# pierreaubert/math-audio

Hardware: NVIDIA B200
Metric: bem_assemble_plus_gmres_seconds_per_frequency (lower is better)
Workload: dtype f64

## Files before the change

### math_audio_b200/csrc/linalg.cu

```cuda
#include <cooperative_groups.h>
#include <atomic>
#include <cstdlib>

#include <string>

#include "linalg.h"

namespace cg = cooperative_groups;

namespace bemb {

constexpr int MAX_DEVICES = 64;
static inline int cur_dev() {
    int d = 0;
    if (cudaGetDevice(&d) != cudaSuccess) { cudaGetLastError(); d = 0; }
    return d >= 0 && d < MAX_DEVICES ? d : MAX_DEVICES - 1;
}
struct PerDeviceFlag {
    std::atomic<unsigned char> v[MAX_DEVICES];
    PerDeviceFlag() { for (auto& x : v) x.store(0); }
    bool get() const { return v[cur_dev()].load() != 0; }
    void set() { v[cur_dev()].store(1); }
};
struct PerDeviceInt {
    std::atomic<int> v[MAX_DEVICES];
    explicit PerDeviceInt(int init) { for (auto& x : v) x.store(init); }
    int get() const { return v[cur_dev()].load(); }
    void set(int val) { v[cur_dev()].store(val); }
};

namespace {

constexpr int GEMV_THREADS = 256;

__device__ __forceinline__ double2 ld_stream(const cplx* p) { return __ldcs(reinterpret_cast<const double2*>(p)); }
__device__ __forceinline__ double2 ld_ro(const cplx* p) { return __ldg(reinterpret_cast<const double2*>(p)); }

__device__ __forceinline__ void cfma(double& are, double& aim, double2 a, double2 x) {
    are = fma(a.x, x.x, are);
    are = fma(-a.y, x.y, are);
    aim = fma(a.x, x.y, aim);
    aim = fma(a.y, x.x, aim);
}

__device__ __forceinline__ unsigned long long global_timer_ns() {
    unsigned long long t;
    asm volatile("mov.u64 %0, %globaltimer;" : "=l"(t));
    return t;
}
__device__ __forceinline__ void ll_store(uint4* dst, double re, double im, uint32_t flag) {
    const uint32_t rl = (uint32_t)__double2loint(re), rh = (uint32_t)__double2hiint(re);
    const uint32_t il = (uint32_t)__double2loint(im), ih = (uint32_t)__double2hiint(im);
    asm volatile("st.volatile.global.v4.u32 [%0], {%1, %2, %3, %4};" ::"l"(dst), "r"(rl), "r"(flag), "r"(rh), "r"(flag) : "memory");
    asm volatile("st.volatile.global.v4.u32 [%0], {%1, %2, %3, %4};" ::"l"(dst + 1), "r"(il), "r"(flag), "r"(ih), "r"(flag) : "memory");
}
template <int N>
__device__ __forceinline__ void ll_load_many(cplx (&out)[N], const uint4* src, uint64_t first, uint64_t stride, uint64_t len,
                                             uint32_t flag, int* err, unsigned long long timeout_ns) {
    bool have[N];
#pragma unroll
    for (int e = 0; e < N; ++e) {
        have[e] = first + (uint64_t)e * stride >= len;
        out[e] = C(0, 0);
    }
    unsigned long long t0 = 0;
    unsigned int spins = 0;
    for (;;) {
        uint4 a[N], b[N];
#pragma unroll
        for (int e = 0; e < N; ++e) {
            if (!have[e]) {
                const uint4* q = src + 2 * (first + (uint64_t)e * stride);
                asm volatile("ld.volatile.global.v4.u32 {%0, %1, %2, %3}, [%4];" : "=r"(a[e].x), "=r"(a[e].y), "=r"(a[e].z), "=r"(a[e].w) : "l"(q) : "memory");
                asm volatile("ld.volatile.global.v4.u32 {%0, %1, %2, %3}, [%4];" : "=r"(b[e].x), "=r"(b[e].y), "=r"(b[e].z), "=r"(b[e].w) : "l"(q + 1) : "memory");
            }
        }
        bool all = true;
#pragma unroll
        for (int e = 0; e < N; ++e) {
            if (!have[e]) {
                if (a[e].y == flag && a[e].w == flag && b[e].y == flag && b[e].w == flag) {
                    have[e] = true;
                    out[e] = C(__hiloint2double((int)a[e].z, (int)a[e].x), __hiloint2double((int)b[e].z, (int)b[e].x));
                } else {
                    all = false;
                }
            }
        }
        if (all) break;
        if ((++spins & 63u) == 0) {
            const unsigned long long t = global_timer_ns();
            if (t0 == 0) t0 = t;
            else if (t - t0 > timeout_ns) {
                *reinterpret_cast<volatile int*>(err) = 1;
                break;
            }
        }
    }
}

template <int GEMV_RB, int GEMV_U, bool FUSED>
__global__ void __launch_bounds__(GEMV_THREADS)
zgemv_kernel(const cplx* __restrict__ A, uint64_t lda, uint64_t nrows, uint64_t ncols, const cplx* __restrict__ x,
             cplx* __restrict__ y, PeerOut po) {
    __shared__ double red[GEMV_RB][2][GEMV_THREADS / 32];
    const int tid = threadIdx.x, lane = tid & 31, warp = tid >> 5;
    for (uint64_t rb = (uint64_t)blockIdx.x * GEMV_RB; rb < nrows; rb += (uint64_t)gridDim.x * GEMV_RB) {
        double are[GEMV_RB], aim[GEMV_RB];
        const cplx* rowp[GEMV_RB];
#pragma unroll
        for (int r = 0; r < GEMV_RB; ++r) {
            are[r] = 0.0; aim[r] = 0.0;
            uint64_t row = rb + r < nrows ? rb + r : nrows - 1;
            rowp[r] = A + row * lda;
        }
        uint64_t c = tid;
        for (; c + (GEMV_U - 1) * GEMV_THREADS < ncols; c += GEMV_U * GEMV_THREADS) {
            double2 a[GEMV_RB][GEMV_U], xv[GEMV_U];
#pragma unroll
            for (int u = 0; u < GEMV_U; ++u) {
#pragma unroll
                for (int r = 0; r < GEMV_RB; ++r) a[r][u] = ld_stream(rowp[r] + c + u * GEMV_THREADS);
                xv[u] = ld_ro(x + c + u * GEMV_THREADS);
            }
#pragma unroll
            for (int u = 0; u < GEMV_U; ++u)
#pragma unroll
                for (int r = 0; r < GEMV_RB; ++r) cfma(are[r], aim[r], a[r][u], xv[u]);
        }
        for (; c < ncols; c += GEMV_THREADS) {
            const double2 x0 = ld_ro(x + c);
#pragma unroll
            for (int r = 0; r < GEMV_RB; ++r) cfma(are[r], aim[r], ld_stream(rowp[r] + c), x0);
        }
#pragma unroll
        for (int r = 0; r < GEMV_RB; ++r) {
#pragma unroll
            for (int m = 16; m >= 1; m >>= 1) {
                are[r] += __shfl_xor_sync(0xffffffffu, are[r], m);
                aim[r] += __shfl_xor_sync(0xffffffffu, aim[r], m);
            }
            if (lane == 0) { red[r][0][warp] = are[r]; red[r][1][warp] = aim[r]; }
        }
        __syncthreads();
        if (tid < GEMV_RB && rb + tid < nrows) {
            double sr = 0.0, si = 0.0;
#pragma unroll
            for (int w = 0; w < GEMV_THREADS / 32; ++w) { sr += red[tid][0][w]; si += red[tid][1][w]; }
            if (FUSED) {
#pragma unroll
                for (int p = 0; p < MAX_PEERS; ++p)
                    if (p < po.npeers) ll_store(po.ll[p] + 2 * (rb + tid), sr, si, po.epoch);
            } else {
                y[rb + tid] = C(sr, si);
            }
        }
        __syncthreads();
    }
}

constexpr int GEMVT_MAX_CHUNKS = 32;
__global__ void __launch_bounds__(256)
zgemv_t_partial_kernel(const cplx* __restrict__ A, uint64_t lda, uint64_t nrows, uint64_t ncols, uint64_t rows_per_chunk,
                       const cplx* __restrict__ x, cplx* __restrict__ part) {
    const uint64_t col = (uint64_t)blockIdx.x * 256 + threadIdx.x;
    const uint64_t r0 = (uint64_t)blockIdx.y * rows_per_chunk;
    const uint64_t r1 = r0 + rows_per_chunk < nrows ? r0 + rows_per_chunk : nrows;
    if (col >= ncols) return;
    double sr = 0.0, si = 0.0;
    for (uint64_t r = r0; r < r1; ++r) cfma(sr, si, ld_stream(A + r * lda + col), ld_ro(x + r));
    part[(uint64_t)blockIdx.y * ncols + col] = C(sr, si);
}
__global__ void __launch_bounds__(256)
zgemv_t_reduce_kernel(const cplx* __restrict__ part, uint64_t ncols, int nchunks, cplx* __restrict__ y) {
    const uint64_t col = (uint64_t)blockIdx.x * 256 + threadIdx.x;
    if (col >= ncols) return;
    double sr = 0.0, si = 0.0;
    for (int c = 0; c < nchunks; ++c) { sr += part[(uint64_t)c * ncols + col].re; si += part[(uint64_t)c * ncols + col].im; }
    y[col] = C(sr, si);
}

constexpr int MAX_CLUSTER = 16;
constexpr int MAX_WARPS = 32;

struct ClusterShared {
    cplx part[2][MAX_CLUSTER * MAX_WARPS];
};

__device__ __forceinline__ cplx cluster_allreduce(cplx v, ClusterShared& sh, int parity) {
    cg::cluster_group cluster = cg::this_cluster();
    const unsigned nb = cluster.num_blocks(), me = cluster.block_rank();
    const unsigned lane = threadIdx.x & 31, warp = threadIdx.x >> 5, nw = blockDim.x >> 5;
#pragma unroll
    for (int m = 16; m >= 1; m >>= 1) {
        v.re += __shfl_xor_sync(0xffffffffu, v.re, m);
        v.im += __shfl_xor_sync(0xffffffffu, v.im, m);
    }
    if (lane < nb) {
        ClusterShared* remote = cluster.map_shared_rank(&sh, lane);
        remote->part[parity][me * nw + warp] = v;
    }
    cluster.sync();
    cplx t = C(0, 0);
    const unsigned total = nb * nw;
    for (unsigned sidx = lane; sidx < total; sidx += 32) {
        t.re += sh.part[parity][sidx].re;
        t.im += sh.part[parity][sidx].im;
    }
#pragma unroll
    for (int m = 16; m >= 1; m >>= 1) {
        t.re += __shfl_xor_sync(0xffffffffu, t.re, m);
        t.im += __shfl_xor_sync(0xffffffffu, t.im, m);
    }
    return t;
}

__device__ __forceinline__ cplx ldg_c(const cplx* p) {
    double2 v = __ldg(reinterpret_cast<const double2*>(p));
    return C(v.x, v.y);
}

template <int EPT>
__global__ void __launch_bounds__(256)
mgs_cluster_reg_kernel(const cplx* __restrict__ V, uint64_t ldv, const cplx* __restrict__ w, int j, uint64_t n, uint64_t S,
                       cplx* __restrict__ hcol, cplx* __restrict__ vnext, double breakdown_tol,
                       const cplx* __restrict__ pinv, int direct_scale) {
    __shared__ ClusterShared sh;
    cg::cluster_group cluster = cg::this_cluster();
    const unsigned me = cluster.block_rank();
    const uint64_t begin = (uint64_t)me * S;
    const uint64_t end = begin + S < n ? begin + S : n;
    const uint64_t len = end > begin ? end - begin : 0;
    cplx wr[EPT], vc[EPT], vn[EPT];
#pragma unroll
    for (int e = 0; e < EPT; ++e) {
        const uint64_t k = threadIdx.x + (uint64_t)e * blockDim.x;
        wr[e] = k < len ? w[begin + k] : C(0, 0);
        if (pinv && k < len) wr[e] = wr[e] * ldg_c(pinv + begin + k);
        vc[e] = k < len ? ldg_c(V + begin + k) : C(0, 0);
    }
    int parity = 0;
    for (int i = 0; i <= j; ++i) {
        if (i < j) {
            const cplx* vi1 = V + (uint64_t)(i + 1) * ldv + begin;
#pragma unroll
            for (int e = 0; e < EPT; ++e) {
                const uint64_t k = threadIdx.x + (uint64_t)e * blockDim.x;
                vn[e] = k < len ? ldg_c(vi1 + k) : C(0, 0);
            }
        }
        cplx acc = C(0, 0);
#pragma unroll
        for (int e = 0; e < EPT; ++e) {
            acc.re = fma(vc[e].re, wr[e].re, fma(vc[e].im, wr[e].im, acc.re));
            acc.im = fma(vc[e].re, wr[e].im, fma(-vc[e].im, wr[e].re, acc.im));
        }
        const cplx h = cluster_allreduce(acc, sh, parity);
        parity ^= 1;
        if (me == 0 && threadIdx.x == 0) hcol[i] = h;
#pragma unroll
        for (int e = 0; e < EPT; ++e) {
            wr[e].re = fma(-h.re, vc[e].re, fma(h.im, vc[e].im, wr[e].re));
            wr[e].im = fma(-h.re, vc[e].im, fma(-h.im, vc[e].re, wr[e].im));
            vc[e] = vn[e];
        }
    }
    cplx acc = C(0, 0);
#pragma unroll
    for (int e = 0; e < EPT; ++e) acc.re = fma(wr[e].re, wr[e].re, fma(wr[e].im, wr[e].im, acc.re));
    const cplx nn = cluster_allreduce(acc, sh, parity);
    const double nrm = sqrt(nn.re);
    if (me == 0 && threadIdx.x == 0) hcol[j + 1] = C(nrm, 0.0);
    if (!(nrm < breakdown_tol)) {
        const double inv = 1.0 / nrm;
        const double sc = inv - 1.0;
#pragma unroll
        for (int e = 0; e < EPT; ++e) {
            const uint64_t k = threadIdx.x + (uint64_t)e * blockDim.x;
            if (k < len)
                vnext[begin + k] = direct_scale ? C(wr[e].re * inv, wr[e].im * inv)
                                                : C(wr[e].re + wr[e].re * sc, wr[e].im + wr[e].im * sc);
        }
    }
    cluster.sync();
}

constexpr int LS_THREADS = 256;
constexpr int LS_WARPS = LS_THREADS / 32;
constexpr int LS_MAXV = 64;

template <int EPT>
__global__ void __launch_bounds__(LS_THREADS)
mgs_lowsync_kernel(const cplx* __restrict__ V, uint64_t ldv, const cplx* __restrict__ w, int j, uint64_t n, uint64_t S,
                   cplx* __restrict__ Lmat, int ldl, cplx* __restrict__ hcol, cplx* __restrict__ vnext, double breakdown_tol,
                   const cplx* __restrict__ pinv, int direct_scale, cplx* __restrict__ hcol_host, PeerWait pw) {
    extern __shared__ __align__(16) unsigned char dyn[];
    __shared__ ClusterShared sh1;
    cplx* warp_part = reinterpret_cast<cplx*>(dyn);
    cplx* slots = warp_part + LS_WARPS * 2 * LS_MAXV;
    cplx* avec = slots + MAX_CLUSTER * 2 * LS_MAXV;
    cplx* Ls = avec + LS_MAXV;
    cg::cluster_group cluster = cg::this_cluster();
    const unsigned nb = cluster.num_blocks(), me = cluster.block_rank();
    const int tid = threadIdx.x, lane = tid & 31, warp = tid >> 5;
    const int nv = j + 1;
    const uint64_t begin = (uint64_t)me * S;
    const uint64_t end = begin + S < n ? begin + S : n;
    const uint64_t len = end > begin ? end - begin : 0;

    cplx wr[EPT], vj[EPT];
    if (pw.ll) ll_load_many<EPT>(wr, pw.ll + 2 * begin, (uint64_t)tid, (uint64_t)LS_THREADS, len, pw.epoch, pw.err, pw.timeout_ns);
#pragma unroll
    for (int e = 0; e < EPT; ++e) {
        const uint64_t k = tid + (uint64_t)e * LS_THREADS;
        if (!pw.ll) wr[e] = k < len ? w[begin + k] : C(0, 0);
        if (pinv && k < len) wr[e] = wr[e] * ldg_c(pinv + begin + k);
        vj[e] = (k < len) ? ldg_c(V + (uint64_t)j * ldv + begin + k) : C(0, 0);
    }
    for (int idx = tid; idx < nv * nv; idx += LS_THREADS) {
        const int k = idx / nv, l = idx - k * nv;
        Ls[idx] = (l < k && k < j) ? Lmat[k * ldl + l] : C(0, 0);
    }

    for (int l0 = 0; l0 < nv; l0 += 8) {
        cplx aa[8], gg[8];
#pragma unroll
        for (int q = 0; q < 8; ++q) { aa[q] = C(0, 0); gg[q] = C(0, 0); }
#pragma unroll
        for (int e = 0; e < EPT; ++e) {
            const uint64_t k = tid + (uint64_t)e * LS_THREADS;
#pragma unroll
            for (int q = 0; q < 8; ++q) {
                const int l = l0 + q;
                const cplx v = (l < nv && k < len) ? ldg_c(V + (uint64_t)l * ldv + begin + k) : C(0, 0);
                aa[q].re = fma(v.re, wr[e].re, fma(v.im, wr[e].im, aa[q].re));
                aa[q].im = fma(v.re, wr[e].im, fma(-v.im, wr[e].re, aa[q].im));
                gg[q].re = fma(vj[e].re, v.re, fma(vj[e].im, v.im, gg[q].re));
                gg[q].im = fma(vj[e].re, v.im, fma(-vj[e].im, v.re, gg[q].im));
            }
        }
#pragma unroll
        for (int q = 0; q < 8; ++q) {
#pragma unroll
            for (int m = 16; m >= 1; m >>= 1) {
                aa[q].re += __shfl_xor_sync(0xffffffffu, aa[q].re, m);
                aa[q].im += __shfl_xor_sync(0xffffffffu, aa[q].im, m);
                gg[q].re += __shfl_xor_sync(0xffffffffu, gg[q].re, m);
                gg[q].im += __shfl_xor_sync(0xffffffffu, gg[q].im, m);
            }
            if (lane == 0 && l0 + q < nv) {
                warp_part[warp * 2 * LS_MAXV + l0 + q] = aa[q];
                warp_part[warp * 2 * LS_MAXV + LS_MAXV + l0 + q] = gg[q];
            }
        }
    }
    __syncthreads();
    if (tid < 2 * nv) {
        const int idx = tid < nv ? tid : LS_MAXV + (tid - nv);
        cplx t = C(0, 0);
#pragma unroll
        for (int wq = 0; wq < LS_WARPS; ++wq) { t.re += warp_part[wq * 2 * LS_MAXV + idx].re; t.im += warp_part[wq * 2 * LS_MAXV + idx].im; }
        for (unsigned d = 0; d < nb; ++d) {
            cplx* remote = cluster.map_shared_rank(slots, d);
            remote[me * 2 * LS_MAXV + idx] = t;
        }
    }
    cluster.sync();
    if (tid < 2 * nv) {
        const int idx = tid < nv ? tid : LS_MAXV + (tid - nv);
        cplx t = C(0, 0);
        for (unsigned d = 0; d < nb; ++d) { t.re += slots[d * 2 * LS_MAXV + idx].re; t.im += slots[d * 2 * LS_MAXV + idx].im; }
        if (tid < nv) {
            avec[tid] = t;
        } else {
            const int l = tid - nv;
            if (l < j) {
                Ls[j * nv + l] = t;
                if (me == 0) Lmat[j * ldl + l] = t;
            }
        }
    }
    __syncthreads();
    if (warp == 0) {
        for (int l = 0; l < nv; ++l) {
            const cplx hl = avec[l];
            for (int k = l + 1 + lane; k < nv; k += 32) {
                const cplx lk = Ls[k * nv + l];
                cplx ak = avec[k];
                ak.re -= lk.re * hl.re - lk.im * hl.im;
                ak.im -= lk.re * hl.im + lk.im * hl.re;
                avec[k] = ak;
            }
            __syncwarp();
        }
        if (me == 0)
            for (int l = lane; l < nv; l += 32) {
                hcol[l] = avec[l];
                if (hcol_host) hcol_host[l] = avec[l];
            }
    }
    __syncthreads();
    for (int l0 = 0; l0 < nv; l0 += 8) {
#pragma unroll
        for (int e = 0; e < EPT; ++e) {
            const uint64_t k = tid + (uint64_t)e * LS_THREADS;
#pragma unroll
            for (int q = 0; q < 8; ++q) {
                const int l = l0 + q;
                if (l < nv && k < len) {
                    const cplx v = ldg_c(V + (uint64_t)l * ldv + begin + k);
                    const cplx h = avec[l];
                    wr[e].re = fma(-h.re, v.re, fma(h.im, v.im, wr[e].re));
                    wr[e].im = fma(-h.re, v.im, fma(-h.im, v.re, wr[e].im));
                }
            }
        }
    }
    cplx acc = C(0, 0);
#pragma unroll
    for (int e = 0; e < EPT; ++e) acc.re = fma(wr[e].re, wr[e].re, fma(wr[e].im, wr[e].im, acc.re));
    const cplx nn = cluster_allreduce(acc, sh1, 0);
    const double nrm = sqrt(nn.re);
    if (me == 0 && tid == 0) {
        hcol[j + 1] = C(nrm, 0.0);
        if (hcol_host) hcol_host[j + 1] = C(nrm, 0.0);
    }
    if (!(nrm < breakdown_tol)) {
        const double inv = 1.0 / nrm;
        const double sc = inv - 1.0;
#pragma unroll
        for (int e = 0; e < EPT; ++e) {
            const uint64_t k = tid + (uint64_t)e * LS_THREADS;
            if (k < len)
                vnext[begin + k] = direct_scale ? C(wr[e].re * inv, wr[e].im * inv)
                                                : C(wr[e].re + wr[e].re * sc, wr[e].im + wr[e].im * sc);
        }
    }
    cluster.sync();
}

constexpr int GR_MAX_CTAS = 148;

__device__ __forceinline__ double warp_reduce32(double (&v)[32], int lane) {
#pragma unroll
    for (int off = 16, cnt = 16; off >= 1; off >>= 1, cnt >>= 1) {
        const bool upper = (lane & off) != 0;
#pragma unroll
        for (int i = 0; i < cnt; ++i) {
            const double send = upper ? v[i] : v[i + cnt];
            const double keep = upper ? v[i + cnt] : v[i];
            v[i] = keep + __shfl_xor_sync(0xffffffffu, send, off);
        }
    }
    return v[0];
}

template <int EPT, int GR_THREADS>
__global__ void __launch_bounds__(GR_THREADS)
mgs_grid_kernel(const cplx* __restrict__ V, uint64_t ldv, const cplx* __restrict__ w, int j, uint64_t n, uint64_t S,
                cplx* __restrict__ Lmat, int ldl, cplx* __restrict__ hcol, cplx* __restrict__ vnext, double breakdown_tol,
// ... 474 lines not shown
#pragma unroll
        for (int t = 0; t < NT; ++t) {
            double4 v = make_double4(acc_re[t][0], acc_im[t][0], acc_re[t][1], acc_im[t][1]);
            *reinterpret_cast<double4*>(yrow + t * 8 + 2 * kq) = v;
        }
    }
}

template <int EPT>
__global__ void __launch_bounds__(256)
mgs_batched_kernel(const cplx* __restrict__ Vall, uint64_t ldv, uint64_t vstride, const cplx* __restrict__ Yblk, int S_rhs,
                   int j, uint64_t n, uint64_t S, cplx* __restrict__ hcol_all, uint64_t hstride, cplx* __restrict__ Xblk,
                   double breakdown_tol, const unsigned char* __restrict__ active) {
    __shared__ ClusterShared sh;
    cg::cluster_group cluster = cg::this_cluster();
    const unsigned me = cluster.block_rank();
    const int rhs = blockIdx.y;
    if (active && !active[rhs]) return;
    const cplx* V = Vall + (uint64_t)rhs * vstride;
    cplx* hcol = hcol_all + (uint64_t)rhs * hstride;
    const uint64_t begin = (uint64_t)me * S;
    const uint64_t end = begin + S < n ? begin + S : n;
    const uint64_t len = end > begin ? end - begin : 0;
    cplx wr[EPT], vc[EPT], vn[EPT];
#pragma unroll
    for (int e = 0; e < EPT; ++e) {
        const uint64_t k = threadIdx.x + (uint64_t)e * blockDim.x;
        wr[e] = k < len ? ldg_c(Yblk + (begin + k) * S_rhs + rhs) : C(0, 0);
        vc[e] = k < len ? ldg_c(V + begin + k) : C(0, 0);
    }
    int parity = 0;
    for (int i = 0; i <= j; ++i) {
        if (i < j) {
            const cplx* vi1 = V + (uint64_t)(i + 1) * ldv + begin;
#pragma unroll
            for (int e = 0; e < EPT; ++e) {
                const uint64_t k = threadIdx.x + (uint64_t)e * blockDim.x;
                vn[e] = k < len ? ldg_c(vi1 + k) : C(0, 0);
            }
        }
        cplx acc = C(0, 0);
#pragma unroll
        for (int e = 0; e < EPT; ++e) {
            acc.re = fma(vc[e].re, wr[e].re, fma(vc[e].im, wr[e].im, acc.re));
            acc.im = fma(vc[e].re, wr[e].im, fma(-vc[e].im, wr[e].re, acc.im));
        }
        const cplx h = cluster_allreduce(acc, sh, parity);
        parity ^= 1;
        if (me == 0 && threadIdx.x == 0) hcol[i] = h;
#pragma unroll
        for (int e = 0; e < EPT; ++e) {
            wr[e].re = fma(-h.re, vc[e].re, fma(h.im, vc[e].im, wr[e].re));
            wr[e].im = fma(-h.re, vc[e].im, fma(-h.im, vc[e].re, wr[e].im));
            vc[e] = vn[e];
        }
    }
    cplx acc = C(0, 0);
#pragma unroll
    for (int e = 0; e < EPT; ++e) acc.re = fma(wr[e].re, wr[e].re, fma(wr[e].im, wr[e].im, acc.re));
    const cplx nn = cluster_allreduce(acc, sh, parity);
    const double nrm = sqrt(nn.re);
    if (me == 0 && threadIdx.x == 0) hcol[j + 1] = C(nrm, 0.0);
    if (!(nrm < breakdown_tol)) {
        const double sc = 1.0 / nrm - 1.0;
        cplx* vnext = const_cast<cplx*>(V) + (uint64_t)(j + 1) * ldv;
#pragma unroll
        for (int e = 0; e < EPT; ++e) {
            const uint64_t k = threadIdx.x + (uint64_t)e * blockDim.x;
            if (k < len) {
                const cplx v = C(wr[e].re + wr[e].re * sc, wr[e].im + wr[e].im * sc);
                vnext[begin + k] = v;
                Xblk[(begin + k) * S_rhs + rhs] = v;
            }
        }
    }
    cluster.sync();
}

__global__ void __launch_bounds__(256)
mgs_batched_smem_kernel(const cplx* __restrict__ Vall, uint64_t ldv, uint64_t vstride, const cplx* __restrict__ Yblk, int S_rhs,
                        int j, uint64_t n, uint64_t S, cplx* __restrict__ hcol_all, uint64_t hstride, cplx* __restrict__ Xblk,
                        double breakdown_tol, const unsigned char* __restrict__ active) {
    extern __shared__ __align__(16) unsigned char mgs_smem_raw[];
    cplx* w_s = reinterpret_cast<cplx*>(mgs_smem_raw);
    __shared__ ClusterShared sh;
    cg::cluster_group cluster = cg::this_cluster();
    const unsigned me = cluster.block_rank();
    const int rhs = blockIdx.y;
    if (active && !active[rhs]) return;
    const cplx* V = Vall + (uint64_t)rhs * vstride;
    cplx* hcol = hcol_all + (uint64_t)rhs * hstride;
    const uint64_t begin = (uint64_t)me * S;
    const uint64_t end = begin + S < n ? begin + S : n;
    const uint64_t len = end > begin ? end - begin : 0;
    for (uint64_t k = threadIdx.x; k < len; k += 256) w_s[k] = ldg_c(Yblk + (begin + k) * S_rhs + rhs);
    int parity = 0;
    for (int i = 0; i <= j; ++i) {
        const cplx* vi = V + (uint64_t)i * ldv + begin;
        cplx acc = C(0, 0);
        for (uint64_t k = threadIdx.x; k < len; k += 256) {
            const cplx v = ldg_c(vi + k), w = w_s[k];
            acc.re = fma(v.re, w.re, fma(v.im, w.im, acc.re));
            acc.im = fma(v.re, w.im, fma(-v.im, w.re, acc.im));
        }
        const cplx h = cluster_allreduce(acc, sh, parity);
        parity ^= 1;
        if (me == 0 && threadIdx.x == 0) hcol[i] = h;
        for (uint64_t k = threadIdx.x; k < len; k += 256) {
            const cplx v = ldg_c(vi + k);
            cplx w = w_s[k];
            w.re = fma(-h.re, v.re, fma(h.im, v.im, w.re));
            w.im = fma(-h.re, v.im, fma(-h.im, v.re, w.im));
            w_s[k] = w;
        }
    }
    cplx acc = C(0, 0);
    for (uint64_t k = threadIdx.x; k < len; k += 256) {
        const cplx w = w_s[k];
        acc.re = fma(w.re, w.re, fma(w.im, w.im, acc.re));
    }
    const cplx nn = cluster_allreduce(acc, sh, parity);
    const double nrm = sqrt(nn.re);
    if (me == 0 && threadIdx.x == 0) hcol[j + 1] = C(nrm, 0.0);
    if (!(nrm < breakdown_tol)) {
        const double sc = 1.0 / nrm - 1.0;
        cplx* vnext = const_cast<cplx*>(V) + (uint64_t)(j + 1) * ldv;
        for (uint64_t k = threadIdx.x; k < len; k += 256) {
            const cplx w = w_s[k];
            const cplx v = C(w.re + w.re * sc, w.im + w.im * sc);
            vnext[begin + k] = v;
            Xblk[(begin + k) * S_rhs + rhs] = v;
        }
    }
    cluster.sync();
}

__global__ void __launch_bounds__(1024)
block_residual_kernel(const cplx* __restrict__ B, const cplx* __restrict__ AX, cplx* __restrict__ R, uint64_t n, int S_rhs,
                      double* __restrict__ out) {
    __shared__ double red[32];
    const int rhs = blockIdx.x;
    double acc = 0.0;
    for (uint64_t k = threadIdx.x; k < n; k += blockDim.x) {
        cplx v = B[k * S_rhs + rhs];
        if (AX) { v.re -= AX[k * S_rhs + rhs].re; v.im -= AX[k * S_rhs + rhs].im; }
        if (R) R[k * S_rhs + rhs] = v;
        acc = fma(v.re, v.re, fma(v.im, v.im, acc));
    }
#pragma unroll
    for (int m = 16; m >= 1; m >>= 1) acc += __shfl_xor_sync(0xffffffffu, acc, m);
    if ((threadIdx.x & 31) == 0) red[threadIdx.x >> 5] = acc;
    __syncthreads();
    if (threadIdx.x == 0) {
        double t = 0.0;
        for (int w = 0; w < (int)(blockDim.x >> 5); ++w) t += red[w];
        out[rhs] = t;
    }
}

__global__ void block_scale_kernel(const cplx* __restrict__ R, const double* __restrict__ scale, cplx* __restrict__ Vall,
                                   uint64_t vstride, cplx* __restrict__ Xblk, uint64_t n, int S_rhs) {
    const uint64_t total = n * (uint64_t)S_rhs;
    for (uint64_t e = (uint64_t)blockIdx.x * blockDim.x + threadIdx.x; e < total; e += (uint64_t)gridDim.x * blockDim.x) {
        const uint64_t k = e / S_rhs;
        const int s = (int)(e - k * S_rhs);
        const double sc = scale[s];
        const cplx v = C(R[e].re * sc, R[e].im * sc);
        Xblk[e] = v;
        Vall[(uint64_t)s * vstride + k] = v;
    }
}

__global__ void block_update_x_kernel(cplx* __restrict__ Xsol, const cplx* __restrict__ Vall, uint64_t ldv, uint64_t vstride,
                                      const cplx* __restrict__ ycoef, int ldy, const int* __restrict__ cnt, uint64_t n, int S_rhs) {
    const uint64_t total = n * (uint64_t)S_rhs;
    for (uint64_t e = (uint64_t)blockIdx.x * blockDim.x + threadIdx.x; e < total; e += (uint64_t)gridDim.x * blockDim.x) {
        const uint64_t k = e / S_rhs;
        const int s = (int)(e - k * S_rhs);
        const int c = cnt[s];
        if (c <= 0) continue;
        cplx v = Xsol[e];
        const cplx* V = Vall + (uint64_t)s * vstride;
        for (int i = 0; i < c; ++i) {
            const cplx a = ycoef[s * ldy + i], b = V[(uint64_t)i * ldv + k];
            v.re += a.re * b.re - a.im * b.im;
            v.im += a.re * b.im + a.im * b.re;
        }
        Xsol[e] = v;
    }
}

__global__ void scale_kernel(const cplx* __restrict__ r, double s, cplx* __restrict__ v, uint64_t n) {
    for (uint64_t k = (uint64_t)blockIdx.x * blockDim.x + threadIdx.x; k < n; k += (uint64_t)gridDim.x * blockDim.x)
        v[k] = C(r[k].re * s, r[k].im * s);
}

__global__ void update_x_kernel(cplx* __restrict__ x, const cplx* __restrict__ V, uint64_t ldv, const cplx* __restrict__ ycoef,
                                int cnt, uint64_t n) {
    for (uint64_t k = (uint64_t)blockIdx.x * blockDim.x + threadIdx.x; k < n; k += (uint64_t)gridDim.x * blockDim.x) {
        cplx v = x[k];
        for (int i = 0; i < cnt; ++i) {
            const cplx a = ycoef[i], b = V[(uint64_t)i * ldv + k];
            v.re += a.re * b.re - a.im * b.im;
            v.im += a.re * b.im + a.im * b.re;
        }
        x[k] = v;
    }
}

__global__ void row_sum_kernel(cplx* __restrict__ A, uint64_t lda, uint64_t nloc, uint64_t ncols, uint64_t r0,
                               cplx* __restrict__ rowsums) {
    const int lane = threadIdx.x & 31;
    const uint64_t row = ((uint64_t)blockIdx.x * blockDim.x + threadIdx.x) >> 5;
    if (row >= nloc) return;
    cplx acc = C(0, 0);
    for (uint64_t c = lane; c < ncols; c += 32) { acc.re += A[row * lda + c].re; acc.im += A[row * lda + c].im; }
#pragma unroll
    for (int m = 16; m >= 1; m >>= 1) {
        acc.re += __shfl_xor_sync(0xffffffffu, acc.re, m);
        acc.im += __shfl_xor_sync(0xffffffffu, acc.im, m);
    }
    if (lane == 0) {
        rowsums[row] = acc;
        A[row * lda + r0 + row].re -= acc.re;
        A[row * lda + r0 + row].im -= acc.im;
    }
}

__global__ void __launch_bounds__(256)
dfma_peak_kernel(double* out, int iters, double a, double b) {
    double x0 = threadIdx.x, x1 = x0 + 1, x2 = x0 + 2, x3 = x0 + 3, x4 = x0 + 4, x5 = x0 + 5, x6 = x0 + 6, x7 = x0 + 7;
    for (int i = 0; i < iters; ++i) {
#pragma unroll
        for (int u = 0; u < 8; ++u) {
            x0 = fma(x0, a, b); x1 = fma(x1, a, b); x2 = fma(x2, a, b); x3 = fma(x3, a, b);
            x4 = fma(x4, a, b); x5 = fma(x5, a, b); x6 = fma(x6, a, b); x7 = fma(x7, a, b);
        }
    }
    double s = x0 + x1 + x2 + x3 + x4 + x5 + x6 + x7;
    if (s == 123.456) out[0] = s;
}

__device__ __forceinline__ void atomic_max_pos(double* addr, double v) {
    atomicMax(reinterpret_cast<unsigned long long*>(addr), (unsigned long long)__double_as_longlong(v));
}
struct SelftestKappas {
    double kap[8];
    CisConst pos[8], neg[8];
};
__global__ void math_selftest_kernel(uint64_t n, double xmax, double* err, SelftestKappas kk) {
    __shared__ double2 tab[SINCOS_TAB];
    for (int i = threadIdx.x; i < SINCOS_TAB; i += blockDim.x) {
        double sv, cv;
        sincospi((double)i / SINCOS_STEPS_PER_PI, &sv, &cv);
        tab[i] = make_double2(cv, sv);
    }
    __syncthreads();
    double e_sc = 0.0, e_rs = 0.0;
    for (uint64_t k = (uint64_t)blockIdx.x * blockDim.x + threadIdx.x; k < n; k += (uint64_t)gridDim.x * blockDim.x) {
        double u = (double)k * 0.6180339887498949;
        u -= floor(u);
        double x = u * xmax;
        double s, c, fs, fc;
        sincos(x, &s, &c);
        fast_sincos(x, fs, fc);
        e_sc = fmax(e_sc, fmax(fabs(fs - s), fabs(fc - c)));
        const int ki = (int)(k & 7);
        const double kap = kk.kap[ki];
        const double r = x / kap;
        const double p = kap * r, e = fma(kap, r, -p);
        sincos(p, &s, &c);
        const double s_ref = fma(e, c, s), c_ref = fma(-e, s, c);
        fast_cis_tab(r, kk.pos[ki], tab, fs, fc);
        e_sc = fmax(e_sc, fmax(fabs(fs - s_ref), fabs(fc - c_ref)));
        fast_cis_tab(r, kk.neg[ki], tab, fs, fc);
        e_sc = fmax(e_sc, fmax(fabs(fs + s_ref), fabs(fc - c_ref)));
        double a = x * x + 1e-12;
        double ref = 1.0 / sqrt(a);
        e_rs = fmax(e_rs, fabs(fast_rsqrt(a) - ref) / ref);
    }
    atomic_max_pos(&err[0], e_sc);
    atomic_max_pos(&err[1], e_rs);
}

template <class Kern, class... Args>
cudaError_t launch_cluster(Kern kern, int cluster, int threads, size_t smem, cudaStream_t s, Args... args) {
    cudaLaunchConfig_t cfg = {};
    cfg.gridDim = dim3(cluster, 1, 1);
    cfg.blockDim = dim3(threads, 1, 1);
    cfg.dynamicSmemBytes = smem;
    cfg.stream = s;
    cudaLaunchAttribute attr[1];
    attr[0].id = cudaLaunchAttributeClusterDimension;
    attr[0].val.clusterDim.x = cluster;
    attr[0].val.clusterDim.y = 1;
    attr[0].val.clusterDim.z = 1;
    cfg.attrs = attr;
    cfg.numAttrs = 1;
    return cudaLaunchKernelEx(&cfg, kern, args...);
}

}

static cudaError_t launch_zgemv_impl(const cplx* A, uint64_t lda, uint64_t nrows, uint64_t ncols, const cplx* x, cplx* y,
                                     const PeerOut* po, cudaStream_t s) {
    if (nrows == 0 && !po) return cudaSuccess;
    static const int variant = []() { const char* v = std::getenv("BEMB200_GEMV_VARIANT"); return v ? std::atoi(v) : 24; }();
    const int rb = variant / 10, u = variant % 10;
    uint64_t blocks = (nrows + rb - 1) / rb;
    const uint64_t maxb = 148ull * 8ull * 8ull;
    if (blocks > maxb) blocks = maxb;
    if (blocks == 0) blocks = 1;
    if (po) {
        zgemv_kernel<2, 4, true><<<(unsigned)((nrows + 1) / 2 > maxb ? maxb : (nrows + 1) / 2 ? (nrows + 1) / 2 : 1), GEMV_THREADS, 0, s>>>(
            A, lda, nrows, ncols, x, y, *po);
        return cudaGetLastError();
    }
    const PeerOut none{};
#define GEMV_CASE(R, U) \
    if (rb == R && u == U) { zgemv_kernel<R, U, false><<<(unsigned)blocks, GEMV_THREADS, 0, s>>>(A, lda, nrows, ncols, x, y, none); return cudaGetLastError(); }
    GEMV_CASE(4, 2) GEMV_CASE(2, 2)
#undef GEMV_CASE
    zgemv_kernel<2, 4, false><<<(unsigned)blocks, GEMV_THREADS, 0, s>>>(A, lda, nrows, ncols, x, y, none);
    return cudaGetLastError();
}

cudaError_t launch_zgemv(const cplx* A, uint64_t lda, uint64_t nrows, uint64_t ncols, const cplx* x, cplx* y, cudaStream_t s) {
    return launch_zgemv_impl(A, lda, nrows, ncols, x, y, nullptr, s);
}

cudaError_t launch_zgemv_peer(const cplx* A, uint64_t lda, uint64_t nrows, uint64_t ncols, const cplx* x, const PeerOut& po,
                              cudaStream_t s) {
    return launch_zgemv_impl(A, lda, nrows, ncols, x, nullptr, &po, s);
}

cudaError_t launch_zgemv_t(const cplx* A, uint64_t lda, uint64_t nrows, uint64_t ncols, const cplx* x, cplx* y, cudaStream_t s) {
    if (nrows == 0) return cudaMemsetAsync(y, 0, ncols * sizeof(cplx), s);
    const uint64_t rpc = (nrows + GEMVT_MAX_CHUNKS - 1) / GEMVT_MAX_CHUNKS;
    const int nchunks = (int)((nrows + rpc - 1) / rpc);
    cplx* part = nullptr;
    cudaError_t e = cudaMallocAsync((void**)&part, (size_t)nchunks * ncols * sizeof(cplx), s);
    if (e != cudaSuccess) return e;
    dim3 grid((unsigned)((ncols + 255) / 256), (unsigned)nchunks);
    zgemv_t_partial_kernel<<<grid, 256, 0, s>>>(A, lda, nrows, ncols, rpc, x, part);
    zgemv_t_reduce_kernel<<<(unsigned)((ncols + 255) / 256), 256, 0, s>>>(part, ncols, nchunks, y);
    e = cudaGetLastError();
    cudaFreeAsync(part, s);
    return e;
}

static int pick_cluster(uint64_t n, int level, bool* w_in_smem, size_t* smem_bytes, uint64_t* slice) {
    int cl = n >= 4096 ? 8 : 1;
    uint64_t S = (n + cl - 1) / cl;
    const size_t cap = 200 * 1024;
    if (level == 0 && S * sizeof(cplx) > cap && cl == 8) {
        cl = 16;
        S = (n + cl - 1) / cl;
    }
    bool fits = level == 0 && S * sizeof(cplx) <= cap;
    *w_in_smem = fits;
    *smem_bytes = fits ? S * sizeof(cplx) : 0;
    *slice = S;
    return cl;
}

static PerDeviceInt g_cluster_level(0);

template <int EPT>
static cudaError_t launch_mgs_reg(int cl, const cplx* V, uint64_t ldv, const cplx* w, int j, uint64_t n, uint64_t S, cplx* hcol,
                                  cplx* vnext, const cplx* pinv, int direct_scale, cudaStream_t s) {
    static PerDeviceFlag attr_done;
    if (!attr_done.get()) {
        cudaError_t e = cudaFuncSetAttribute(mgs_cluster_reg_kernel<EPT>, cudaFuncAttributeNonPortableClusterSizeAllowed, 1);
        if (e != cudaSuccess) return e;
        attr_done.set();
    }
    return launch_cluster(mgs_cluster_reg_kernel<EPT>, cl, 256, 0, s, V, ldv, w, j, n, S, hcol, vnext, 1e-14, pinv, direct_scale);
}

template <int EPT>
static cudaError_t launch_mgs_lowsync(int cl, const cplx* V, uint64_t ldv, const cplx* w, int j, uint64_t n, uint64_t S, cplx* Lmat,
                                      int ldl, cplx* hcol, cplx* vnext, const cplx* pinv, int direct_scale, cplx* hcol_host,
                                      const PeerWait& pw, cudaStream_t s) {
    static PerDeviceFlag attr_done;
    const size_t fixed = (size_t)(LS_WARPS * 2 * LS_MAXV + MAX_CLUSTER * 2 * LS_MAXV + LS_MAXV) * sizeof(cplx);
    if (!attr_done.get()) {
        cudaError_t e = cudaFuncSetAttribute(mgs_lowsync_kernel<EPT>, cudaFuncAttributeNonPortableClusterSizeAllowed, 1);
        if (e != cudaSuccess) return e;
        e = cudaFuncSetAttribute(mgs_lowsync_kernel<EPT>, cudaFuncAttributeMaxDynamicSharedMemorySize,
                                 (int)(fixed + (size_t)LS_MAXV * LS_MAXV * sizeof(cplx)));
        if (e != cudaSuccess) return e;
        attr_done.set();
    }
    const size_t smem = fixed + (size_t)(j + 1) * (j + 1) * sizeof(cplx);
    return launch_cluster(mgs_lowsync_kernel<EPT>, cl, LS_THREADS, smem, s, V, ldv, w, j, n, S, Lmat, ldl, hcol, vnext, 1e-14, pinv,
                          direct_scale, hcol_host, pw);
}

template <int EPT, int GR_THREADS>
static cudaError_t launch_mgs_grid(int G, const cplx* V, uint64_t ldv, const cplx* w, int j, uint64_t n, uint64_t S, cplx* Lmat,
                                   int ldl, cplx* hcol, cplx* vnext, const cplx* pinv, int direct_scale, cplx* scratch,
                                   cplx* hcol_host, const PeerWait& pw, cudaStream_t s) {
    constexpr int GR_WARPS = GR_THREADS / 32;
    static PerDeviceFlag attr_done;
    const size_t fixed = (size_t)(GR_WARPS * 2 * LS_MAXV + LS_MAXV) * sizeof(cplx);
    if (!attr_done.get()) {
        cudaError_t e = cudaFuncSetAttribute(mgs_grid_kernel<EPT, GR_THREADS>, cudaFuncAttributeMaxDynamicSharedMemorySize,
                                             (int)(fixed + (size_t)LS_MAXV * LS_MAXV * sizeof(cplx)));
        if (e != cudaSuccess) return e;
        attr_done.set();
    }
    cudaLaunchConfig_t cfg = {};
    cfg.gridDim = dim3(G, 1, 1);
    cfg.blockDim = dim3(GR_THREADS, 1, 1);
    cfg.dynamicSmemBytes = fixed + (size_t)(j + 1) * (j + 1) * sizeof(cplx);
    cfg.stream = s;
    cudaLaunchAttribute attr[1];
    attr[0].id = cudaLaunchAttributeCooperative;
    attr[0].val.cooperative = 1;
    cfg.attrs = attr;
    cfg.numAttrs = 1;
    cplx* part = scratch;
    double* npart = reinterpret_cast<double*>(scratch + (size_t)GR_MAX_CTAS * 2 * LS_MAXV);
    const double tol = 1e-14;
    return cudaLaunchKernelEx(&cfg, mgs_grid_kernel<EPT, GR_THREADS>, V, ldv, w, j, n, S, Lmat, ldl, hcol, vnext, tol, pinv, direct_scale,
                              part, npart, hcol_host, pw);
}

size_t mgs_scratch_elems() { return (size_t)GR_MAX_CTAS * 2 * LS_MAXV + GR_MAX_CTAS; }

static const int g_mgs_mode_env = []() {
    const char* v = std::getenv("BEMB200_MGS_MODE");
    return v ? std::atoi(v) : 3;
}();
static PerDeviceInt g_mgs_mode(g_mgs_mode_env);

bool mgs_peer_wait_capable(uint64_t n, uint32_t restart, bool allow_grid) {
    if (restart + 1 > (uint32_t)LS_MAXV) return false;
    const int mode = g_mgs_mode.get();
    if (mode != 3 && mode != 0) return false;
    if (n <= 16ull * LS_THREADS * 8ull) return true;
    return mode == 3 && allow_grid && n <= (uint64_t)GR_MAX_CTAS * 1024ull;
}

static cudaError_t launch_mgs_cluster_path(int mode_in, const cplx* V, uint64_t ldv, cplx* w, int j, uint64_t n, cplx* hcol,
                                           cplx* vnext, const cplx* pinv, int direct_scale, cplx* Lmat, int ldl, cplx* hcol_host,
                                           bool* wrote_host, const PeerWait& pw, bool strict, cudaStream_t s) {
    *wrote_host = false;
    static PerDeviceInt cluster_mode(-1);
    if (cluster_mode.get() < 0) cluster_mode.set(mode_in);
    int mode = cluster_mode.get();
    if (mode == 0 && Lmat && j + 1 <= LS_MAXV && n <= 16ull * LS_THREADS * 8ull) {
        const int cl = n >= 2048 ? 16 : (n >= 512 ? 4 : 1);
        const uint64_t S = (n + cl - 1) / cl;
        const uint64_t ept = (S + LS_THREADS - 1) / LS_THREADS;
        cudaError_t e;
        if (ept <= 1) e = launch_mgs_lowsync<1>(cl, V, ldv, w, j, n, S, Lmat, ldl, hcol, vnext, pinv, direct_scale, hcol_host, pw, s);
        else if (ept <= 2) e = launch_mgs_lowsync<2>(cl, V, ldv, w, j, n, S, Lmat, ldl, hcol, vnext, pinv, direct_scale, hcol_host, pw, s);
        else if (ept <= 4) e = launch_mgs_lowsync<4>(cl, V, ldv, w, j, n, S, Lmat, ldl, hcol, vnext, pinv, direct_scale, hcol_host, pw, s);
        else e = launch_mgs_lowsync<8>(cl, V, ldv, w, j, n, S, Lmat, ldl, hcol, vnext, pinv, direct_scale, hcol_host, pw, s);
        if (e == cudaSuccess) { *wrote_host = hcol_host != nullptr; return e; }
        if (strict) return e;
        cudaGetLastError();
        mode = 2;
        cluster_mode.set(mode);
    }
    if (pw.ll) return cudaErrorNotSupported;
    if ((mode == 0 || mode == 2) && n <= 16ull * 256ull * 8ull) {
        const int cl = n >= 2048 ? 16 : (n >= 512 ? 4 : 1);
        const uint64_t S = (n + cl - 1) / cl;
        const uint64_t ept = (S + 255) / 256;
        cudaError_t e;
        if (ept <= 1) e = launch_mgs_reg<1>(cl, V, ldv, w, j, n, S, hcol, vnext, pinv, direct_scale, s);
        else if (ept <= 2) e = launch_mgs_reg<2>(cl, V, ldv, w, j, n, S, hcol, vnext, pinv, direct_scale, s);
        else if (ept <= 4) e = launch_mgs_reg<4>(cl, V, ldv, w, j, n, S, hcol, vnext, pinv, direct_scale, s);
        else e = launch_mgs_reg<8>(cl, V, ldv, w, j, n, S, hcol, vnext, pinv, direct_scale, s);
        if (e == cudaSuccess) return e;
        if (strict) return e;
        cudaGetLastError();
        cluster_mode.set(1);
    }
    static PerDeviceFlag attr_done;
    if (!attr_done.get()) {
        cudaError_t e = cudaFuncSetAttribute(mgs_cluster_kernel, cudaFuncAttributeMaxDynamicSharedMemorySize, 200 * 1024);
        if (e != cudaSuccess) return e;
        e = cudaFuncSetAttribute(mgs_cluster_kernel, cudaFuncAttributeNonPortableClusterSizeAllowed, 1);
        if (e != cudaSuccess) return e;
        attr_done.set();
    }
    for (;;) {
        bool in_smem;
        size_t smem;
        uint64_t S;
        const int level = strict ? 1 : g_cluster_level.get();
        int cl = pick_cluster(n, level, &in_smem, &smem, &S);
        cudaError_t e = launch_cluster(mgs_cluster_kernel, cl, VEC_THREADS, smem, s, V, ldv, w, j, n, S, (int)in_smem, hcol,
                                       vnext, 1e-14, pinv, direct_scale);
        if (e == cudaSuccess || level == 1) return e;
        cudaGetLastError();
        g_cluster_level.set(1);
    }
}

cudaError_t launch_mgs(const cplx* V, uint64_t ldv, cplx* w, int j, uint64_t n, cplx* hcol, cplx* vnext, const cplx* pinv,
                       int direct_scale, cplx* Lmat, int ldl, cplx* scratch, cplx* hcol_host, bool* wrote_host, bool allow_grid,
                       const PeerWait& pw, bool strict, cudaStream_t s) {
    *wrote_host = false;
    static const bool force_grid = []() { const char* v = std::getenv("BEMB200_MGS_FORCE_GRID"); return v ? std::atoi(v) != 0 : true; }();
    const int mode = g_mgs_mode.get();
    if (mode == 3 && (allow_grid || force_grid) && Lmat && scratch && j + 1 <= LS_MAXV && n >= 4096 && n <= (uint64_t)GR_MAX_CTAS * 1024ull) {
        const int G = GR_MAX_CTAS;
        const uint64_t S = (n + G - 1) / G;
        cudaError_t e;
#define GRID_CASE(E, T) e = launch_mgs_grid<E, T>(G, V, ldv, w, j, n, S, Lmat, ldl, hcol, vnext, pinv, direct_scale, scratch, hcol_host, pw, s)
        if (S <= 128) GRID_CASE(1, 128);
        else if (S <= 256) GRID_CASE(2, 128);
        else if (S <= 512) GRID_CASE(2, 256);
        else GRID_CASE(4, 256);
#undef GRID_CASE
        if (e == cudaSuccess) { *wrote_host = hcol_host != nullptr; return e; }
        if (strict) return e;
        cudaGetLastError();
        g_mgs_mode.set(0);
    }
    const int m2 = g_mgs_mode.get();
    return launch_mgs_cluster_path(m2 == 3 ? 0 : m2, V, ldv, w, j, n, hcol, vnext, pinv, direct_scale, Lmat, ldl,
                                   hcol_host, wrote_host, pw, strict, s);
}

cudaError_t launch_residual(const cplx* b, const cplx* ax, cplx* r, uint64_t n, double* out, const cplx* pinv, cudaStream_t s) {
    bool in_smem;
    size_t smem;
    uint64_t S;
    int cl = pick_cluster(n, 1, &in_smem, &smem, &S);
    return launch_cluster(residual_cluster_kernel, cl, VEC_THREADS, 0, s, b, ax, r, n, S, out, pinv);
}

static inline int bicg_cluster(uint64_t n, uint64_t* S) {
    const int cl = n >= 4096 ? 8 : 1;
    *S = (n + cl - 1) / cl;
    return cl;
}
cudaError_t launch_bicg_dot(const cplx* a, const cplx* b, uint64_t n, cplx* out, cudaStream_t s) {
    uint64_t S;
    const int cl = bicg_cluster(n, &S);
    return launch_cluster(bicg_dot_kernel, cl, VEC_THREADS, 0, s, a, b, n, S, out);
}
cudaError_t launch_bicg_p(const cplx* r, cplx* p, const cplx* v, cplx beta, cplx omega, uint64_t n, cudaStream_t s) {
    bicg_p_kernel<<<(unsigned)((n + 255) / 256), 256, 0, s>>>(r, p, v, beta, omega, n);
    return cudaGetLastError();
}
cudaError_t launch_bicg_s(const cplx* r, const cplx* v, cplx alpha, cplx* sv, uint64_t n, cplx* out, cudaStream_t s) {
    uint64_t S;
    const int cl = bicg_cluster(n, &S);
    return launch_cluster(bicg_s_kernel, cl, VEC_THREADS, 0, s, r, v, alpha, sv, n, S, out);
}
cudaError_t launch_bicg_tt(const cplx* t, const cplx* sv, uint64_t n, cplx* out, cudaStream_t s) {
    uint64_t S;
    const int cl = bicg_cluster(n, &S);
    return launch_cluster(bicg_tt_kernel, cl, VEC_THREADS, 0, s, t, sv, n, S, out);
}
cudaError_t launch_bicg_update(cplx* x, const cplx* p, const cplx* sv, const cplx* t, cplx* r, const cplx* r0, cplx alpha, cplx omega,
                               uint64_t n, cplx* out, cudaStream_t s) {
    uint64_t S;
    const int cl = bicg_cluster(n, &S);
    return launch_cluster(bicg_update_kernel, cl, VEC_THREADS, 0, s, x, p, sv, t, r, r0, alpha, omega, n, S, out);
}
cudaError_t launch_bicg_axpy(cplx* x, const cplx* p, cplx alpha, uint64_t n, cudaStream_t s) {
    bicg_axpy_kernel<<<(unsigned)((n + 255) / 256), 256, 0, s>>>(x, p, alpha, n);
    return cudaGetLastError();
}

cudaError_t launch_cgs_q(const cplx* u, const cplx* v, cplx alpha, cplx* q, cplx* uq, uint64_t n, cudaStream_t s) {
    cgs_q_kernel<<<(unsigned)((n + 255) / 256), 256, 0, s>>>(u, v, alpha, q, uq, n);
    return cudaGetLastError();
}
cudaError_t launch_cgs_update(cplx* x, const cplx* uq, const cplx* w, cplx* r, const cplx* r0, cplx alpha, uint64_t n, cplx* out,
                              cudaStream_t s) {
    uint64_t S;
    const int cl = bicg_cluster(n, &S);
    return launch_cluster(cgs_update_kernel, cl, VEC_THREADS, 0, s, x, uq, w, r, r0, alpha, n, S, out);
}
cudaError_t launch_cgs_p(const cplx* r, const cplx* q, cplx beta, cplx* u, cplx* p, uint64_t n, cudaStream_t s) {
    cgs_p_kernel<<<(unsigned)((n + 255) / 256), 256, 0, s>>>(r, q, beta, u, p, n);
    return cudaGetLastError();
}

cudaError_t launch_zgemm_block(const cplx* A, uint64_t lda, uint64_t nrows, uint64_t ncols, const cplx* X, cplx* Y, int nrhs,
                               cudaStream_t s) {
    if (nrows == 0) return cudaSuccess;
    static const bool use_dmma = []() { const char* v = std::getenv("BEMB200_BLOCK_MATVEC"); return v && std::string(v) == "legacy"; }();
    if (!use_dmma) return launch_zgemm_block_streamk(A, lda, nrows, ncols, X, Y, nrhs, s);
    const unsigned blocks = (unsigned)((nrows + BM_ROWS - 1) / BM_ROWS);
    switch (nrhs) {
        case 8: zgemm_block_kernel<1><<<blocks, BM_WARPS * 32, 0, s>>>(A, lda, nrows, ncols, X, Y); break;
        case 16: zgemm_block_kernel<2><<<blocks, BM_WARPS * 32, 0, s>>>(A, lda, nrows, ncols, X, Y); break;
        case 24: zgemm_block_kernel<3><<<blocks, BM_WARPS * 32, 0, s>>>(A, lda, nrows, ncols, X, Y); break;
        case 32: zgemm_block_kernel<4><<<blocks, BM_WARPS * 32, 0, s>>>(A, lda, nrows, ncols, X, Y); break;
        default: return cudaErrorInvalidValue;
    }
    return cudaGetLastError();
}

template <int EPT>
static cudaError_t launch_mgs_batched_t(int cl, int nrhs, const cplx* Vall, uint64_t ldv, uint64_t vstride, const cplx* Yblk,
                                        int j, uint64_t n, uint64_t S, cplx* hcol_all, uint64_t hstride, cplx* Xblk,
                                        const unsigned char* active, cudaStream_t s) {
    static PerDeviceFlag attr_done;
    if (!attr_done.get()) {
        cudaError_t e = cudaFuncSetAttribute(mgs_batched_kernel<EPT>, cudaFuncAttributeNonPortableClusterSizeAllowed, 1);
        if (e != cudaSuccess) return e;
// ... 129 lines not shown
```

Baseline: 0.1094.

## Add TMA bulk-copy pipelined complex GEMV kernel with warp-specialized producer

```diff
diff --git a/math_audio_b200/csrc/linalg.cu b/math_audio_b200/csrc/linalg.cu
--- a/math_audio_b200/csrc/linalg.cu
+++ b/math_audio_b200/csrc/linalg.cu
@@ -156,6 +156,121 @@
             }
         }
         __syncthreads();
+    }
+}
+
+constexpr int GEMV_BULK_RB = 2, GEMV_BULK_CC = 1024, GEMV_BULK_S = 3;
+constexpr int GEMV_BULK_THREADS = GEMV_THREADS + 32;
+constexpr size_t GEMV_BULK_SMEM = (size_t)GEMV_BULK_S * GEMV_BULK_RB * GEMV_BULK_CC * sizeof(cplx);
+
+__device__ __forceinline__ uint32_t smem_addr(const void* p) { return (uint32_t)__cvta_generic_to_shared(p); }
+__device__ __forceinline__ void mbar_init(uint64_t* bar, uint32_t count) {
+    asm volatile("mbarrier.init.shared::cta.b64 [%0], %1;" ::"r"(smem_addr(bar)), "r"(count) : "memory");
+}
+__device__ __forceinline__ void mbar_wait(uint64_t* bar, uint32_t parity) {
+    uint32_t done = 0;
+    while (!done)
+        asm volatile("{\n .reg .pred p;\n mbarrier.try_wait.parity.shared::cta.b64 p, [%1], %2;\n selp.u32 %0, 1, 0, p;\n}"
+                     : "=r"(done) : "r"(smem_addr(bar)), "r"(parity) : "memory");
+}
+__device__ __forceinline__ void mbar_arrive(uint64_t* bar) {
+    asm volatile("mbarrier.arrive.shared::cta.b64 _, [%0];" ::"r"(smem_addr(bar)) : "memory");
+}
+__device__ __forceinline__ void mbar_arrive_expect_tx(uint64_t* bar, uint32_t bytes) {
+    asm volatile("mbarrier.arrive.expect_tx.shared::cta.b64 _, [%0], %1;" ::"r"(smem_addr(bar)), "r"(bytes) : "memory");
+}
+__device__ __forceinline__ void bulk_load(void* dst, const void* src, uint32_t bytes, uint64_t* bar, uint64_t policy) {
+    asm volatile("cp.async.bulk.shared::cta.global.mbarrier::complete_tx::bytes.L2::cache_hint [%0], [%1], %2, [%3], %4;"
+                 ::"r"(smem_addr(dst)), "l"(src), "r"(bytes), "r"(smem_addr(bar)), "l"(policy) : "memory");
+}
+
+template <int RB, int CC, int S>
+__global__ void __launch_bounds__(GEMV_BULK_THREADS, 1)
+zgemv_bulk_kernel(const cplx* __restrict__ A, uint64_t lda, uint64_t nrows, uint64_t ncols, const cplx* __restrict__ x,
+                  cplx* __restrict__ y) {
+    static_assert(CC % GEMV_THREADS == 0, "a stage must keep thread t on the columns = t (mod 256)");
+    constexpr int NW = GEMV_THREADS / 32, CPT = CC / GEMV_THREADS;
+    extern __shared__ __align__(128) double2 ring[];
+    __shared__ __align__(8) uint64_t full[S], empty[S];
+    __shared__ double red[2][RB][2][NW];
+    const int tid = threadIdx.x, lane = tid & 31, warp = tid >> 5;
+    if (tid == 0) {
+        for (int s = 0; s < S; ++s) { mbar_init(&full[s], 1); mbar_init(&empty[s], NW); }
+        asm volatile("fence.mbarrier_init.release.cluster;" ::: "memory");
+    }
+    __syncthreads();
+    const uint64_t nblk = (nrows + RB - 1) / RB, nchunks = (ncols + CC - 1) / CC;
+    int stage = 0;
+    uint32_t phase = 0;
+    if (warp == NW) {
+        if (lane != 0) return;
+        uint64_t policy;
+        asm volatile("createpolicy.fractional.L2::evict_first.b64 %0, 1.0;" : "=l"(policy));
+        for (uint64_t b = blockIdx.x; b < nblk; b += gridDim.x) {
+            const uint64_t r0 = b * RB;
+            const int nr = nrows - r0 < (uint64_t)RB ? (int)(nrows - r0) : RB;
+            for (uint64_t c0 = 0; c0 < ncols; c0 += CC) {
+                const uint32_t bytes = (uint32_t)((ncols - c0 < (uint64_t)CC ? ncols - c0 : (uint64_t)CC) * sizeof(cplx));
+                mbar_wait(&empty[stage], phase ^ 1);
+                mbar_arrive_expect_tx(&full[stage], bytes * (uint32_t)nr);
+                for (int r = 0; r < nr; ++r) bulk_load(ring + (stage * RB + r) * CC, A + (r0 + r) * lda + c0, bytes, &full[stage], policy);
+                if (++stage == S) { stage = 0; phase ^= 1; }
+            }
+        }
+        return;
+    }
+    double2 xv[CPT];
+    auto load_x = [&](uint64_t c0) {
+#pragma unroll
+        for (int k = 0; k < CPT; ++k) {
+            const uint64_t c = c0 + tid + k * GEMV_THREADS;
+            xv[k] = c < ncols ? ld_ro(x + c) : make_double2(0.0, 0.0);
+        }
+    };
+    load_x(0);
+    int par = 0;
+    for (uint64_t b = blockIdx.x; b < nblk; b += gridDim.x, par ^= 1) {
+        const uint64_t r0 = b * RB;
+        const int nr = nrows - r0 < (uint64_t)RB ? (int)(nrows - r0) : RB;
+        double are[RB], aim[RB];
+#pragma unroll
+        for (int r = 0; r < RB; ++r) { are[r] = 0.0; aim[r] = 0.0; }
+        for (uint64_t ch = 0; ch < nchunks; ++ch) {
+            const uint64_t c0 = ch * CC;
+            double2 xc[CPT];
+#pragma unroll
+            for (int k = 0; k < CPT; ++k) xc[k] = xv[k];
+            load_x(ch + 1 < nchunks ? c0 + CC : 0);
+            mbar_wait(&full[stage], phase);
+            const double2* st = ring + stage * RB * CC;
+#pragma unroll
+            for (int k = 0; k < CPT; ++k) {
+                if (c0 + tid + k * GEMV_THREADS < ncols) {
+#pragma unroll
+                    for (int r = 0; r < RB; ++r)
+                        if (r < nr) cfma(are[r], aim[r], st[r * CC + tid + k * GEMV_THREADS], xc[k]);
+                }
+            }
+            __syncwarp();
+            if (lane == 0) mbar_arrive(&empty[stage]);
+            if (++stage == S) { stage = 0; phase ^= 1; }
+        }
+#pragma unroll
+        for (int r = 0; r < RB; ++r) {
+#pragma unroll
+            for (int m = 16; m >= 1; m >>= 1) {
+                are[r] += __shfl_xor_sync(0xffffffffu, are[r], m);
+                aim[r] += __shfl_xor_sync(0xffffffffu, aim[r], m);
+            }
+            if (lane == 0) { red[par][r][0][warp] = are[r]; red[par][r][1][warp] = aim[r]; }
+        }
+        asm volatile("bar.sync 1, %0;" ::"n"(GEMV_THREADS) : "memory");
+        if (tid < nr) {
+            double sr = 0.0, si = 0.0;
+#pragma unroll
+            for (int w = 0; w < NW; ++w) { sr += red[par][tid][0][w]; si += red[par][tid][1][w]; }
+            y[r0 + tid] = C(sr, si);
+        }
     }
 }
 
@@ -1236,11 +1351,41 @@
 
 }
 
+template <int RB, int CC, int S>
+static cudaError_t launch_zgemv_bulk(const cplx* A, uint64_t lda, uint64_t nrows, uint64_t ncols, const cplx* x, cplx* y, int per_sm,
+                                     cudaStream_t s) {
+    constexpr size_t smem = (size_t)S * RB * CC * sizeof(cplx);
+    static PerDeviceInt sms(0);
+    if (sms.get() == 0) {
+        cudaError_t e = cudaFuncSetAttribute(zgemv_bulk_kernel<RB, CC, S>, cudaFuncAttributeMaxDynamicSharedMemorySize, (int)smem);
+        if (e == cudaSuccess)
+            e = cudaFuncSetAttribute(zgemv_bulk_kernel<RB, CC, S>, cudaFuncAttributePreferredSharedMemoryCarveout, (int)cudaSharedmemCarveoutMaxShared);
+        int n = 0;
+        if (e == cudaSuccess) e = cudaDeviceGetAttribute(&n, cudaDevAttrMultiProcessorCount, cur_dev());
+        if (e != cudaSuccess) return e;
+        sms.set(n);
+    }
+    const uint64_t nblk = (nrows + RB - 1) / RB, g = (uint64_t)sms.get() * per_sm;
+    zgemv_bulk_kernel<RB, CC, S><<<(unsigned)(nblk < g ? nblk : g), GEMV_BULK_THREADS, smem, s>>>(A, lda, nrows, ncols, x, y);
+    return cudaGetLastError();
+}
+
 static cudaError_t launch_zgemv_impl(const cplx* A, uint64_t lda, uint64_t nrows, uint64_t ncols, const cplx* x, cplx* y,
                                      const PeerOut* po, cudaStream_t s) {
     if (nrows == 0 && !po) return cudaSuccess;
-    static const int variant = []() { const char* v = std::getenv("BEMB200_GEMV_VARIANT"); return v ? std::atoi(v) : 24; }();
-    const int rb = variant / 10, u = variant % 10;
+    static const int variant = []() { const char* v = std::getenv("BEMB200_GEMV_VARIANT"); return v ? std::atoi(v) : 0; }();
+    if (!po && variant == 0) {
+        static const int cfg = []() { const char* v = std::getenv("BEMB200_BULK_CFG"); return v ? std::atoi(v) : 0; }();
+        static const int per_sm = []() { const char* v = std::getenv("BEMB200_BULK_CTAS"); return v ? std::atoi(v) : 1; }();
+        switch (cfg) {
+            case 1: return launch_zgemv_bulk<2, 512, 6>(A, lda, nrows, ncols, x, y, per_sm, s);
+            case 2: return launch_zgemv_bulk<2, 512, 8>(A, lda, nrows, ncols, x, y, per_sm, s);
+            case 3: return launch_zgemv_bulk<2, 1024, 4>(A, lda, nrows, ncols, x, y, per_sm, s);
+            case 4: return launch_zgemv_bulk<2, 256, 12>(A, lda, nrows, ncols, x, y, per_sm, s);
+            default: return launch_zgemv_bulk<2, 1024, 3>(A, lda, nrows, ncols, x, y, per_sm, s);
+        }
+    }
+    const int rb = variant / 10 == 4 ? 4 : 2, u = variant % 10;
     uint64_t blocks = (nrows + rb - 1) / rb;
     const uint64_t maxb = 148ull * 8ull * 8ull;
     if (blocks > maxb) blocks = maxb;
```

Measured after the change: 0.1231, median of 6. 1.13x slower.
